# tudelft-iv/instance_stixels

Measured on NVIDIA B200. Metric: stixel frames/sec @1024x2048, higher is better.
Workload: dtype f32

## Files before the change

instance_stixels_b200/csrc/tables.cu:

```cuda
#include <cstdlib>
#include "kernels.h"

namespace isx {

namespace {

__global__ void frame_tables_kernel(const float *__restrict__ ground, const int *__restrict__ vhor_arr,
                                    float *__restrict__ stat, KParams p) {
  const int f = blockIdx.y;
  const int vB = blockIdx.x * blockDim.x + threadIdx.x;
  const int H = p.rows;
  if (vB >= H) return;
  float *S = stat + ((size_t)f * H + vB) * kStatWords;
  if (vB == 0) {
    for (int i = 0; i < kStatWords; i++) S[i] = 0.0f;
    return;
  }
  const float *gf = ground + (size_t)f * 3 * H;
  const int vhor = vhor_arr[f];
  const int pv = vB - 1;
  const float eps = p.epsilon;

  const float pc = ffma(lg2_approx((float)(H - vB)), kLn2, -0.0f);
  const float fnp = clamp_neg(gf[pv]);
  const float t1_hi = fadd(fnp, eps);
  const float t1_lo = fsub(fnp, eps);
  const float og_base = fadd(pc, kNegLog07);
  const float tr1_hi = fadd(neg_log_div(p.pgrav, fsub(fadd(-fnp, p.max_disf), eps)), og_base);
  const float tr1_mid = fadd(neg_log_div(fsub(fadd(-p.pgrav, 1.0f), p.pblg), fadd(eps, eps)), og_base);
  const float tr1_lo = fadd(neg_log_div(p.pblg, t1_lo), og_base);
  const float sky_fg = (gf[pv] < 1.0f) ? pc : inf_f();
  const float oo_base = fadd(pc, (pv < vhor) ? kNegLog07 : kLn2);
  const float tr3 = fadd(pc, ffma(lg2_approx(fsub(p.max_disf, eps)), kLn2, -0.0f));
  const float g_prev = ffma(-kLn2, kLg2_03, pc);
  const float sky_fo = ffma(kLn2, 1.0f, pc);
  S[0] = pc;  S[1] = t1_hi;  S[2] = t1_lo;  S[3] = tr1_hi;  S[4] = tr1_mid;  S[5] = tr1_lo;
  S[6] = sky_fg;  S[7] = oo_base;  S[8] = tr3;  S[9] = g_prev;  S[10] = sky_fo;  S[11] = 0.0f;
}

template <bool TALL>
__device__ void blelloch_prefix_warp(const float *e, int H, float *ps) {
  const unsigned full = 0xffffffffu;
  const int lane = threadIdx.x & 31;
  const int nchunks = (H + 31) >> 5;
  float total_k = 0.0f;
  float total2_k = 0.0f;
  for (int k = 0; k < nchunks; k++) {
    const int v = (k << 5) + lane;
    float x = v < H ? e[v] : 0.0f;
#pragma unroll
    for (int b = 0; b < 5; b++) x = fadd(x, __shfl_xor_sync(full, x, 1 << b));
    if constexpr (TALL) {
      if (lane == (k & 31)) {
        if (k < 32) total_k = x;
        else total2_k = x;
      }
    } else {
      if (lane == k) total_k = x;
    }
  }
  float y = total_k, left[5];
#pragma unroll
  for (int b = 0; b < 5; b++) {
    const float o = __shfl_xor_sync(full, y, 1 << b);
    left[b] = o;
    y = fadd(y, o);
  }
  float hi = 0.0f;
#pragma unroll
  for (int b = 4; b >= 0; b--)
    if ((lane >> b) & 1) hi = fadd(hi, left[b]);
  float hi2 = 0.0f;
  if constexpr (TALL) {
    float y2 = total2_k, left2[5];
#pragma unroll
    for (int b = 0; b < 5; b++) {
      const float o = __shfl_xor_sync(full, y2, 1 << b);
      left2[b] = o;
      y2 = fadd(y2, o);
    }
    hi2 = fadd(0.0f, y);
#pragma unroll
    for (int b = 4; b >= 0; b--)
      if ((lane >> b) & 1) hi2 = fadd(hi2, left2[b]);
  }
  const int kmax = H >> 5;
  for (int k = 0; k <= kmax; k++) {
    const int v = (k << 5) + lane;
    float x = v < H ? e[v] : 0.0f;
    float lo[5];
#pragma unroll
    for (int b = 0; b < 5; b++) {
      const float o = __shfl_xor_sync(full, x, 1 << b);
      lo[b] = o;
      x = fadd(x, o);
    }
    float pre;
    if constexpr (TALL) {
      pre = __shfl_sync(full, k < 32 ? hi : hi2, k & 31);
    } else {
      pre = (k < 32) ? __shfl_sync(full, hi, k & 31) : y;
    }
#pragma unroll
    for (int b = 4; b >= 0; b--)
      if ((lane >> b) & 1) pre = fadd(pre, lo[b]);
    if (v <= H) ps[v] = pre;
  }
}

template <typename T>
__device__ void exact_prefix_warp(const T *e, int n, T *ps) {
  const unsigned full = 0xffffffffu;
  const int lane = threadIdx.x & 31;
  T carry = 0;
  for (int base = 0; base < n; base += 32) {
    const int i = base + lane;
    T x = i < n ? e[i] : (T)0;
    T incl = x;
#pragma unroll
    for (int d = 1; d < 32; d <<= 1) {
      const T o = __shfl_up_sync(full, incl, d);
      if (lane >= d) incl += o;
    }
    if (i < n) ps[i] = carry + incl - x;
    carry += __shfl_sync(full, incl, 31);
  }
  if (lane == 0) ps[n] = carry;
}

constexpr int kTabThreads = 256;

struct TabSmem {
  int Hp, nq;
  size_t off_e[4], off_seg, off_i64, off_i32, total;
  __host__ __device__ TabSmem(int H, int hs2) {
    Hp = (H + 1 + 3) & ~3;
    nq = H / 8 + 1;
    size_t o = 0;
    off_i64 = o; o += (size_t)Hp * 8 * 2;
    off_i32 = o; o += (size_t)Hp * 4 * 2;
    for (int i = 0; i < 4; i++) { off_e[i] = o; o += (size_t)Hp * 4; }
    off_seg = o; o += (size_t)20 * (nq + 1) * 4;
    total = (o + 15) & ~(size_t)15;
    (void)hs2;
  }
};

template <bool TALL> struct TabLimits {
  static constexpr int kMeanRowLimit = TALL ? 1 << 19 : 1 << 20;
  static constexpr int kClassLimit = TALL ? 1 << 19 : 1 << 20;
  static constexpr int kSqOffLimit = TALL ? 1 << 18 : 1 << 19;
};

template <bool TALL>
__global__ void __launch_bounds__(kTabThreads, 4)
column_tables_kernel(const float *__restrict__ joined, const int32_t *__restrict__ segmentation,
                     const float *__restrict__ ground, const int *__restrict__ vhor_arr,
                     uint32_t *__restrict__ records_b, int *__restrict__ error_flag, int *__restrict__ col_flags,
                     KParams p) {
  extern __shared__ __align__(16) unsigned char smem[];
  const int H = p.rows, C = p.realcols;
  const int col = blockIdx.x, f = blockIdx.y;
  const int tid = threadIdx.x, warp = tid >> 5, lane = tid & 31;
  const TabSmem L(H, p.hs2);
  float *e_disp = reinterpret_cast<float *>(smem + L.off_e[0]);
  float *e_valid = reinterpret_cast<float *>(smem + L.off_e[1]);
  float *e_ground = reinterpret_cast<float *>(smem + L.off_e[2]);
  float *e_sky = reinterpret_cast<float *>(smem + L.off_e[3]);
  long long *ps_i64 = reinterpret_cast<long long *>(smem + L.off_i64);
  int *ps_i32 = reinterpret_cast<int *>(smem + L.off_i32);
  int *seg_ps = reinterpret_cast<int *>(smem + L.off_seg);
  const int nq = L.nq, segld = nq + 1;

  const float *d_col = joined + ((size_t)f * C + col) * H;
  const int32_t *seg_col = segmentation + ((size_t)f * C + col) * p.n_channels * p.hs2;
  const float *gf = ground + (size_t)f * 3 * H;
  const float *norm_g = gf + H, *inv_g = gf + 2 * H;
  const int vhor = vhor_arr[f];
  const float invalid = p.invalid_disparity;
  const int K = p.n_classes;
  const bool has_oy = K < p.n_channels, has_ox = K + 1 < p.n_channels;
  constexpr int kMeanRowLimit = TabLimits<TALL>::kMeanRowLimit;

  bool negative_class_value = false;
#pragma unroll
  for (int c = warp; c < 20; c += kTabThreads / 32) {
#pragma unroll 5
    for (int q = lane; q < nq; q += 32) {
      int v = 0;
      if (c < K) {
        if (c < p.n_channels && q < p.hs2) v = __ldg(seg_col + (size_t)c * p.hs2 + q);
        negative_class_value |= v < 0 || v > TabLimits<TALL>::kClassLimit;
      } else {
        int oy = 0, ox = 0;
        if (q < p.hs2 && has_oy) oy = __ldg(seg_col + (size_t)K * p.hs2 + q);
        if (q < p.hs2 && has_ox) ox = __ldg(seg_col + (size_t)(K + 1) * p.hs2 + q);
        oy = oy * oy;
        ox = ox * ox;
        negative_class_value |= oy < 0 || oy > TabLimits<TALL>::kSqOffLimit || ox < 0 ||
                                ox > TabLimits<TALL>::kSqOffLimit;
        v = oy + ox;
      }
      seg_ps[c * segld + q] = v;
    }
  }
  bool out_of_range = false;
  for (int v0 = tid; v0 < H; v0 += 4 * kTabThreads) {
    float d4[4], g0[4], gi[4], gn[4];
    int oy4[4], ox4[4];
#pragma unroll
    for (int j = 0; j < 4; j++) {
      const int v = v0 + j * kTabThreads;
      const bool ok = v < H;
      const int q = v / kDownsample;
      d4[j] = ok ? __ldg(d_col + v) : 0.0f;
      oy4[j] = (ok && q < p.hs2 && has_oy) ? __ldg(seg_col + (size_t)K * p.hs2 + q) : 0;
      ox4[j] = (ok && q < p.hs2 && has_ox) ? __ldg(seg_col + (size_t)(K + 1) * p.hs2 + q) : 0;
      const bool gr = ok && v < vhor;
      g0[j] = gr ? __ldg(gf + v) : 0.0f;
      gi[j] = gr ? __ldg(inv_g + v) : 0.0f;
      gn[j] = gr ? __ldg(norm_g + v) : 0.0f;
    }
#pragma unroll
    for (int j = 0; j < 4; j++) {
      const int v = v0 + j * kTabThreads;
      if (v >= H) break;
      const float d = d4[j];
      if (invalid >= 0.0f) {
        const int va = d != invalid;
        e_valid[v] = (float)va;
        e_disp[v] = fmul((float)va, d);
      } else {
        e_valid[v] = 1.0f;
        e_disp[v] = d;
      }
      float sky = 0.0f;
      if (v >= vhor) {
        sky = p.pnexists_given_sky_log;
        if (d != invalid) {
          const float g = ffma(fmul(d, d), p.inv_sigma2_sky, p.normalization_sky);
          sky = fadd(fmin_(g, p.puniform_sky), p.nopnexists_given_sky_log);
        }
      }
      e_sky[v] = sky;
      float grd = inf_f();
      if (v < vhor) {
        grd = p.pnexists_given_ground_log;
        if (d != invalid) {
          const float diff = fsub(d, g0[j]);
          const float g = ffma(fmul(diff, diff), gi[j], gn[j]);
          grd = fadd(fmin_(g, p.puniform), p.nopnexists_given_ground_log);
        }
      }
      e_ground[v] = grd;
      const long long mx = (long long)((p.column_step * col + 0.5 * (p.column_step - 1.0)) + ox4[j] + 0.5);
      const long long my = (long long)(v - oy4[j] + 0.5);
      out_of_range |= mx <= -kMeanRowLimit || mx >= kMeanRowLimit || my <= -kMeanRowLimit || my >= kMeanRowLimit;
      ps_i32[0 * L.Hp + v] = (int)mx;
      ps_i32[1 * L.Hp + v] = (int)my;
      ps_i64[0 * L.Hp + v] = mx * mx;
      ps_i64[1 * L.Hp + v] = my * my;
    }
  }
  const int any_negative = __syncthreads_or(negative_class_value ? 1 : 0);
  if (tid == 0) col_flags[(size_t)f * C + col] = any_negative;

  if (warp < 4) {
    blelloch_prefix_warp<TALL>(e_disp + warp * L.Hp, H, e_disp + warp * L.Hp);
  } else if (warp < 6) {
    exact_prefix_warp<long long>(ps_i64 + (warp - 4) * L.Hp, H, ps_i64 + (warp - 4) * L.Hp);
  } else {
    exact_prefix_warp<int>(ps_i32 + (warp - 6) * L.Hp, H, ps_i32 + (warp - 6) * L.Hp);
  }
  for (int c = 19 - ((warp + 4) & 7); c >= 0; c -= kTabThreads / 32)
    exact_prefix_warp<int>(seg_ps + c * segld, nq, seg_ps + c * segld);
  __syncthreads();

  uint4 *recb_col = reinterpret_cast<uint4 *>(records_b + ((size_t)f * C + col) * (size_t)p.rec_stride * kRecBWords);
  const long long lim2 = 1ll << (24 + kSqSplitBits);
  const int lim1 = 1 << 24;
  const long long lomask = (1ll << kSqSplitBits) - 1;
  const int g = tid & 7, r = (tid >> 3) & 7;
  const int *ps_grp = seg_ps + (4 * (g < 5 ? g : 4)) * segld;
  const long long *ps_sq = ps_i64 + (g == 5 ? 0 : L.Hp);
  const float *pf_a = g == 6 ? e_disp : e_ground, *pf_b = g == 6 ? e_valid : e_sky;
#pragma unroll 2
  for (int v = tid >> 3; v <= H; v += kTabThreads / 8) {
    uint4 w;
    {
      const int *ps = ps_grp + (v >> 3);
      const int a0 = ps[0], a1 = ps[segld], a2 = ps[2 * segld], a3 = ps[3 * segld];
      w.x = (uint32_t)(a0 * kDownsample + (ps[1] - a0) * r);
      w.y = (uint32_t)(a1 * kDownsample + (ps[segld + 1] - a1) * r);
      w.z = (uint32_t)(a2 * kDownsample + (ps[2 * segld + 1] - a2) * r);
      w.w = (uint32_t)(a3 * kDownsample + (ps[3 * segld + 1] - a3) * r);
    }
    if (g >= 5) {
      const int smx = ps_i32[0 * L.Hp + v], smy = ps_i32[1 * L.Hp + v];
      const long long sq = ps_sq[v];
      out_of_range |= (g == 5 && (smx <= -lim1 || smx >= lim1 || smy <= -lim1 || smy >= lim1)) || (g != 7 && sq >= lim2);
      const float hi = (float)(sq & ~lomask), lo = (float)(sq & lomask);
      const float fa = pf_a[v], fb = pf_b[v];
      w.x = __float_as_uint(g == 5 ? (float)smx : g == 6 ? hi : fa);
      w.y = __float_as_uint(g == 5 ? (float)smy : g == 6 ? lo : fb);
      w.z = g == 7 ? 0u : __float_as_uint(g == 5 ? hi : fa);
      w.w = g == 7 ? 0u : __float_as_uint(g == 5 ? lo : fb);
    }
    recb_col[v * (kRecBWords / 4) + g] = w;
  }
  if (out_of_range) atomicOr(error_flag + f, kErrOffsetRange);
}

constexpr int kLutWarps = 4;
constexpr int kLutThreads = kLutWarps * 32;

__device__ __forceinline__ float ldg_lo_hi(unsigned lo, unsigned hi) {
  float r;
  asm("{\n\t.reg .b64 a;\n\tmov.b64 a, {%1, %2};\n\tld.global.nc.f32 %0, [a];\n\t}" : "=f"(r) : "r"(lo), "r"(hi));
  return r;
}
__device__ __forceinline__ void stg_lo_hi(unsigned lo, unsigned hi, float v) {
  asm volatile("{\n\t.reg .b64 a;\n\tmov.b64 a, {%0, %1};\n\tst.global.f32 [a], %2;\n\t}" ::"r"(lo), "r"(hi), "f"(v)
               : "memory");
}

template <int MAXH>
__global__ void __launch_bounds__(kLutThreads)
object_lut_kernel(const float *__restrict__ joined, const float *__restrict__ cost_t,
                  float *__restrict__ object_lut, KParams p) {
  __shared__ __align__(16) uint8_t dis_s[MAXH + 32];
  __shared__ float tile[kLutWarps][32][33];
  const int H = p.rows, C = p.realcols, D = p.max_dis;
  const int Dp = (D + 31) & ~31;
  const int col = blockIdx.x, f = blockIdx.z;
  const int warp = threadIdx.x >> 5, lane = threadIdx.x & 31;
  const float *d_col = joined + ((size_t)f * C + col) * H;
  const int Hc = (H + 31) & ~31;
  for (int v = threadIdx.x; v < Hc; v += kLutThreads) {
    int di = 0;
    if (v < H) {
      di = (int)d_col[v];
      di = di < 0 ? 0 : (di >= D ? D - 1 : di);
    }
    dis_s[v] = (uint8_t)di;
  }
  __syncthreads();
  const int fn0 = (blockIdx.y * kLutWarps + warp) * 32;
  if (fn0 >= D) return;
  const unsigned long long lut_addr = lut_column_address((unsigned long long)object_lut, (size_t)f * C + col,
                                                         p.lut_cols, (size_t)D * p.lut_stride * 4);
  const unsigned lut_hi = (unsigned)(lut_addr >> 32);
  const unsigned stride4 = (unsigned)p.lut_stride * 4u;
  const unsigned long long cost_addr = (unsigned long long)(cost_t + fn0 + lane);
  const unsigned cost_lo = (unsigned)cost_addr, cost_hi = (unsigned)(cost_addr >> 32);
  const unsigned row4 = (unsigned)Dp * 4u;
  float(*tl)[33] = tile[warp];
  const bool full = fn0 + 32 <= D;
  float carry = 0.0f;
  for (int i = 0; i < Hc; i += 32) {
    float x[32];
    const uint4 *dq = reinterpret_cast<const uint4 *>(dis_s + i);
    const uint4 d0 = dq[0], d1 = dq[1];
    const uint32_t dw[8] = {d0.x, d0.y, d0.z, d0.w, d1.x, d1.y, d1.z, d1.w};
#pragma unroll
    for (int r = 0; r < 32; r++) {
      const unsigned dis = __byte_perm(dw[r >> 2], 0u, 0x4440u | (unsigned)(r & 3));
      x[r] = ldg_lo_hi(dis * row4 + cost_lo, cost_hi);
    }
    x[0] = fadd(x[0], carry);
#pragma unroll
    for (int j = 1; j < 32; j <<= 1) {
#pragma unroll
      for (int L = 31; L >= j; L--) x[L] = fadd(x[L], x[L - j]);
    }
    carry = x[31];
    __syncwarp();
#pragma unroll
    for (int r = 0; r < 32; r++) tl[lane][r] = x[r];
    __syncwarp();
    const int v = i + lane;
    if (v < H) {
      unsigned lo = (unsigned)lut_addr + (unsigned)fn0 * stride4 + 4u * (unsigned)v;
      if (full) {
#pragma unroll
        for (int r = 0; r < 32; r++) {
          stg_lo_hi(lo, lut_hi, tl[r][lane]);
          lo += stride4;
        }
      } else {
#pragma unroll
        for (int r = 0; r < 32; r++) {
          if (fn0 + r < D) stg_lo_hi(lo, lut_hi, tl[r][lane]);
          lo += stride4;
        }
      }
    }
  }
}

}

void launch_frame_tables(const KParams &p, const BatchBuffers &b, int nframes, cudaStream_t s) {
  dim3 grid((p.rows + 255) / 256, nframes);
  frame_tables_kernel<<<grid, 256, 0, s>>>(b.ground, b.vhor, b.stat, p);
  g_launch_count++;
}

static size_t tab_smem_bytes(const KParams &p) { return TabSmem(p.rows, p.hs2).total; }

static size_t padded_smem(size_t need, size_t static_bytes) {
  static const int n = [] {
    const char *e = std::getenv("ISX_TAB_CTAS_PER_SM");
    return e ? std::atoi(e) : 0;
  }();
  if (n <= 0) return need;
  const size_t per_cta = (size_t)(227 * 1024) / (size_t)(n + 1) + 1024;
  const size_t want = per_cta > static_bytes + 1024 ? per_cta - static_bytes - 1024 : 0;
  return want > need ? want : need;
}

template <bool TALL>
static void launch_column_tables_rows(const KParams &p, const BatchBuffers &b, int nframes, cudaStream_t s) {
  constexpr int kLutMaxH = TALL ? 2048 : 1024;
  dim3 grid(p.realcols, nframes);
  const size_t smem = padded_smem(tab_smem_bytes(p), 0);
  static SmemOptIn optin, optin_lut;
  opt_in_smem(column_tables_kernel<TALL>, optin);
  opt_in_smem(object_lut_kernel<kLutMaxH>, optin_lut);
  column_tables_kernel<TALL><<<grid, kTabThreads, smem, s>>>(b.joined, b.segmentation, b.ground, b.vhor, b.records_b,
                                                              b.error_flag, b.col_flags, p);
  dim3 lgrid(p.realcols, (p.max_dis + 32 * kLutWarps - 1) / (32 * kLutWarps), nframes);
  object_lut_kernel<kLutMaxH><<<lgrid, kLutThreads, padded_smem(0, sizeof(float) * kLutWarps * 32 * 33 + kLutMaxH + 32), s>>>(
      b.joined, b.obj_cost_lut_t, b.object_lut, p);
  g_launch_count += 2;
}

void launch_column_tables(const KParams &p, const BatchBuffers &b, int nframes, cudaStream_t s) {
  if (p.rows > kShortRows) launch_column_tables_rows<true>(p, b, nframes, s);
  else launch_column_tables_rows<false>(p, b, nframes, s);
}

}
```

Baseline: 8238.

## Stage record writes via smem and vectorize object LUT stores with chunked tiles

The column tables kernel now assigns one warp per record word group. Each warp computes values for 32 rows, writes them to a swizzled shared-memory staging buffer, then writes them out as contiguous uint4 stores, which should coalesce record writes and cut branch divergence. The object LUT kernel buffers 4 chunks of 32 rows in a larger dynamic shared tile, so each lane can emit float4 global stores instead of scalar ones. The costs are two block-wide syncs per 32-row block, a larger shared footprint that may lower occupancy, and a scalar fallback path for row tails.

Result: no change. 8244, median of 6 (+0.1%).

```diff
diff --git a/instance_stixels_b200/csrc/tables.cu b/instance_stixels_b200/csrc/tables.cu
--- a/instance_stixels_b200/csrc/tables.cu
+++ b/instance_stixels_b200/csrc/tables.cu
@@ -130,9 +130,10 @@
 
 constexpr int kTabThreads = 256;
 
+constexpr int kRecBlockRows = 32;
 struct TabSmem {
   int Hp, nq;
-  size_t off_e[4], off_seg, off_i64, off_i32, total;
+  size_t off_e[4], off_seg, off_i64, off_i32, off_stage, total;
   __host__ __device__ TabSmem(int H, int hs2) {
     Hp = (H + 1 + 3) & ~3;
     nq = H / 8 + 1;
@@ -141,6 +142,8 @@
     off_i32 = o; o += (size_t)Hp * 4 * 2;
     for (int i = 0; i < 4; i++) { off_e[i] = o; o += (size_t)Hp * 4; }
     off_seg = o; o += (size_t)20 * (nq + 1) * 4;
+    o = (o + 15) & ~(size_t)15;
+    off_stage = o; o += (size_t)kRecBlockRows * kRecBWords * 4;
     total = (o + 15) & ~(size_t)15;
     (void)hs2;
   }
@@ -276,43 +279,56 @@
     exact_prefix_warp<int>(seg_ps + c * segld, nq, seg_ps + c * segld);
   __syncthreads();
 
+  static_assert(kTabThreads / 32 * 4 == kRecBWords && kTabThreads / 8 == kRecBlockRows, "one thread per word group");
   uint4 *recb_col = reinterpret_cast<uint4 *>(records_b + ((size_t)f * C + col) * (size_t)p.rec_stride * kRecBWords);
+  uint4 *stage = reinterpret_cast<uint4 *>(smem + L.off_stage);
   const long long lim2 = 1ll << (24 + kSqSplitBits);
   const int lim1 = 1 << 24;
   const long long lomask = (1ll << kSqSplitBits) - 1;
-  const int g = tid & 7, r = (tid >> 3) & 7;
-  const int *ps_grp = seg_ps + (4 * (g < 5 ? g : 4)) * segld;
-  const long long *ps_sq = ps_i64 + (g == 5 ? 0 : L.Hp);
-  const float *pf_a = g == 6 ? e_disp : e_ground, *pf_b = g == 6 ? e_valid : e_sky;
-#pragma unroll 2
-  for (int v = tid >> 3; v <= H; v += kTabThreads / 8) {
+  const int srow = tid >> 3, sgrp = tid & 7;
+  const int *ps_grp = seg_ps + 4 * warp * segld;
+  for (int v0 = 0; v0 <= H; v0 += kRecBlockRows) {
+    const int v = min(v0 + lane, H);
     uint4 w;
-    {
+    if (warp < 5) {
       const int *ps = ps_grp + (v >> 3);
+      const int r = v & 7;
       const int a0 = ps[0], a1 = ps[segld], a2 = ps[2 * segld], a3 = ps[3 * segld];
       w.x = (uint32_t)(a0 * kDownsample + (ps[1] - a0) * r);
       w.y = (uint32_t)(a1 * kDownsample + (ps[segld + 1] - a1) * r);
       w.z = (uint32_t)(a2 * kDownsample + (ps[2 * segld + 1] - a2) * r);
       w.w = (uint32_t)(a3 * kDownsample + (ps[3 * segld + 1] - a3) * r);
-    }
-    if (g >= 5) {
+    } else if (warp == 5) {
       const int smx = ps_i32[0 * L.Hp + v], smy = ps_i32[1 * L.Hp + v];
-      const long long sq = ps_sq[v];
-      out_of_range |= (g == 5 && (smx <= -lim1 || smx >= lim1 || smy <= -lim1 || smy >= lim1)) || (g != 7 && sq >= lim2);
-      const float hi = (float)(sq & ~lomask), lo = (float)(sq & lomask);
-      const float fa = pf_a[v], fb = pf_b[v];
-      w.x = __float_as_uint(g == 5 ? (float)smx : g == 6 ? hi : fa);
-      w.y = __float_as_uint(g == 5 ? (float)smy : g == 6 ? lo : fb);
-      w.z = g == 7 ? 0u : __float_as_uint(g == 5 ? hi : fa);
-      w.w = g == 7 ? 0u : __float_as_uint(g == 5 ? lo : fb);
-    }
-    recb_col[v * (kRecBWords / 4) + g] = w;
+      const long long sq = ps_i64[0 * L.Hp + v];
+      out_of_range |= smx <= -lim1 || smx >= lim1 || smy <= -lim1 || smy >= lim1 || sq >= lim2;
+      w.x = __float_as_uint((float)smx);
+      w.y = __float_as_uint((float)smy);
+      w.z = __float_as_uint((float)(sq & ~lomask));
+      w.w = __float_as_uint((float)(sq & lomask));
+    } else if (warp == 6) {
+      const long long sq = ps_i64[1 * L.Hp + v];
+      out_of_range |= sq >= lim2;
+      w.x = __float_as_uint((float)(sq & ~lomask));
+      w.y = __float_as_uint((float)(sq & lomask));
+      w.z = __float_as_uint(e_disp[v]);
+      w.w = __float_as_uint(e_valid[v]);
+    } else {
+      w = make_uint4(__float_as_uint(e_ground[v]), __float_as_uint(e_sky[v]), 0u, 0u);
+    }
+    stage[lane * 8 + (warp ^ (lane & 7))] = w;
+    __syncthreads();
+    if (v0 + srow <= H) recb_col[(v0 + srow) * (kRecBWords / 4) + sgrp] = stage[srow * 8 + (sgrp ^ (srow & 7))];
+    __syncthreads();
   }
   if (out_of_range) atomicOr(error_flag + f, kErrOffsetRange);
 }
 
 constexpr int kLutWarps = 4;
 constexpr int kLutThreads = kLutWarps * 32;
+constexpr int kLutChunks = 4;
+constexpr int kLutTileLd = 32 * kLutChunks + 4;
+constexpr size_t kLutTileBytes = sizeof(float) * kLutWarps * 32 * kLutTileLd;
 
 __device__ __forceinline__ float ldg_lo_hi(unsigned lo, unsigned hi) {
   float r;
@@ -321,6 +337,11 @@
 }
 __device__ __forceinline__ void stg_lo_hi(unsigned lo, unsigned hi, float v) {
   asm volatile("{\n\t.reg .b64 a;\n\tmov.b64 a, {%0, %1};\n\tst.global.f32 [a], %2;\n\t}" ::"r"(lo), "r"(hi), "f"(v)
+               : "memory");
+}
+__device__ __forceinline__ void stg4_lo_hi(unsigned lo, unsigned hi, float4 v) {
+  asm volatile("{\n\t.reg .b64 a;\n\tmov.b64 a, {%0, %1};\n\tst.global.v4.f32 [a], {%2, %3, %4, %5};\n\t}" ::"r"(lo),
+               "r"(hi), "f"(v.x), "f"(v.y), "f"(v.z), "f"(v.w)
                : "memory");
 }
 
@@ -329,7 +350,7 @@
 object_lut_kernel(const float *__restrict__ joined, const float *__restrict__ cost_t,
                   float *__restrict__ object_lut, KParams p) {
   __shared__ __align__(16) uint8_t dis_s[MAXH + 32];
-  __shared__ float tile[kLutWarps][32][33];
+  extern __shared__ __align__(16) float lut_tile[];
   const int H = p.rows, C = p.realcols, D = p.max_dis;
   const int Dp = (D + 31) & ~31;
   const int col = blockIdx.x, f = blockIdx.z;
@@ -354,47 +375,59 @@
   const unsigned long long cost_addr = (unsigned long long)(cost_t + fn0 + lane);
   const unsigned cost_lo = (unsigned)cost_addr, cost_hi = (unsigned)(cost_addr >> 32);
   const unsigned row4 = (unsigned)Dp * 4u;
-  float(*tl)[33] = tile[warp];
+  float *tl = lut_tile + warp * 32 * kLutTileLd;
   const bool full = fn0 + 32 <= D;
   float carry = 0.0f;
-  for (int i = 0; i < Hc; i += 32) {
-    float x[32];
-    const uint4 *dq = reinterpret_cast<const uint4 *>(dis_s + i);
-    const uint4 d0 = dq[0], d1 = dq[1];
-    const uint32_t dw[8] = {d0.x, d0.y, d0.z, d0.w, d1.x, d1.y, d1.z, d1.w};
-#pragma unroll
-    for (int r = 0; r < 32; r++) {
-      const unsigned dis = __byte_perm(dw[r >> 2], 0u, 0x4440u | (unsigned)(r & 3));
-      x[r] = ldg_lo_hi(dis * row4 + cost_lo, cost_hi);
-    }
-    x[0] = fadd(x[0], carry);
-#pragma unroll
-    for (int j = 1; j < 32; j <<= 1) {
-#pragma unroll
-      for (int L = 31; L >= j; L--) x[L] = fadd(x[L], x[L - j]);
-    }
-    carry = x[31];
+  for (int i0 = 0; i0 < Hc; i0 += 32 * kLutChunks) {
+    const int nc = min(kLutChunks, (Hc - i0) >> 5);
+#pragma unroll 1
+    for (int c = 0; c < nc; c++) {
+      const int i = i0 + 32 * c;
+      float x[32];
+      const uint4 *dq = reinterpret_cast<const uint4 *>(dis_s + i);
+      const uint4 d0 = dq[0], d1 = dq[1];
+      const uint32_t dw[8] = {d0.x, d0.y, d0.z, d0.w, d1.x, d1.y, d1.z, d1.w};
+#pragma unroll
+      for (int r = 0; r < 32; r++) {
+        const unsigned dis = __byte_perm(dw[r >> 2], 0u, 0x4440u | (unsigned)(r & 3));
+        x[r] = ldg_lo_hi(dis * row4 + cost_lo, cost_hi);
+      }
+      x[0] = fadd(x[0], carry);
+#pragma unroll
+      for (int j = 1; j < 32; j <<= 1) {
+#pragma unroll
+        for (int L = 31; L >= j; L--) x[L] = fadd(x[L], x[L - j]);
+      }
+      carry = x[31];
+      float4 *trow = reinterpret_cast<float4 *>(tl + lane * kLutTileLd + 32 * c);
+#pragma unroll
+      for (int k = 0; k < 8; k++) trow[k] = make_float4(x[4 * k], x[4 * k + 1], x[4 * k + 2], x[4 * k + 3]);
+    }
     __syncwarp();
-#pragma unroll
-    for (int r = 0; r < 32; r++) tl[lane][r] = x[r];
-    __syncwarp();
-    const int v = i + lane;
-    if (v < H) {
-      unsigned lo = (unsigned)lut_addr + (unsigned)fn0 * stride4 + 4u * (unsigned)v;
+    const int v = i0 + 4 * lane;
+    unsigned lo = (unsigned)lut_addr + (unsigned)fn0 * stride4 + 4u * (unsigned)v;
+    const float *tv = tl + 4 * lane;
+    if (v + 4 <= H) {
       if (full) {
 #pragma unroll
         for (int r = 0; r < 32; r++) {
-          stg_lo_hi(lo, lut_hi, tl[r][lane]);
+          stg4_lo_hi(lo, lut_hi, *reinterpret_cast<const float4 *>(tv + r * kLutTileLd));
           lo += stride4;
         }
       } else {
 #pragma unroll
         for (int r = 0; r < 32; r++) {
-          if (fn0 + r < D) stg_lo_hi(lo, lut_hi, tl[r][lane]);
+          if (fn0 + r < D) stg4_lo_hi(lo, lut_hi, *reinterpret_cast<const float4 *>(tv + r * kLutTileLd));
           lo += stride4;
         }
       }
-    }
+    } else if (v < H) {
+      for (int r = 0; r < 32 && fn0 + r < D; r++) {
+        for (int k = 0; k < H - v; k++) stg_lo_hi(lo + 4u * k, lut_hi, tv[r * kLutTileLd + k]);
+        lo += stride4;
+      }
+    }
+    __syncwarp();
   }
 }
 
@@ -430,7 +463,7 @@
   column_tables_kernel<TALL><<<grid, kTabThreads, smem, s>>>(b.joined, b.segmentation, b.ground, b.vhor, b.records_b,
                                                               b.error_flag, b.col_flags, p);
   dim3 lgrid(p.realcols, (p.max_dis + 32 * kLutWarps - 1) / (32 * kLutWarps), nframes);
-  object_lut_kernel<kLutMaxH><<<lgrid, kLutThreads, padded_smem(0, sizeof(float) * kLutWarps * 32 * 33 + kLutMaxH + 32), s>>>(
+  object_lut_kernel<kLutMaxH><<<lgrid, kLutThreads, padded_smem(kLutTileBytes, kLutMaxH + 32), s>>>(
       b.joined, b.obj_cost_lut_t, b.object_lut, p);
   g_launch_count += 2;
 }
```
